# TiloccaS/DASemanticSegmentationAML

Measured on NVIDIA B200. Metric: da_train_step_img_per_s, higher is better.
Workload: dtype bf16

## Files before the change

dasemanticsegmentationaml_b200/csrc/igemm.cu:

```cuda
#include <stdlib.h>
#include <string.h>
#include <mutex>

#include "igemm.cuh"
#include "ptx.cuh"
#include "status.h"
#include "b200seg.h"

namespace b200 {

constexpr int kThreads = 192;
constexpr int kMaxStages = 8;

struct PipeBarriers {
  uint64_t full[kMaxStages];
  uint64_t empty[kMaxStages];
  uint64_t accum;
  uint32_t tmem_base;
};

__device__ __forceinline__ float apply_act(float v, int act, float slope) {
  if (act == 1) return fmaxf(v, 0.f);
  if (act == 2) return fmaf(slope, fminf(v, 0.f), fmaxf(v, 0.f));
  return v;
}

__device__ __forceinline__ void store16(const ConvParams& p, size_t off, const float (&v)[16]) {
  if (p.out_f32) {
    float* o = reinterpret_cast<float*>(p.out) + off;
    if (p.wide) {
#pragma unroll
      for (int h = 0; h < 2; ++h) {
        uint32_t r[8];
#pragma unroll
        for (int j = 0; j < 8; ++j) r[j] = __float_as_uint(v[8 * h + j]);
        st_global_v8(o + 8 * h, r);
      }
    } else {
#pragma unroll
      for (int j = 0; j < 4; ++j)
        reinterpret_cast<float4*>(o)[j] = make_float4(v[4 * j], v[4 * j + 1], v[4 * j + 2], v[4 * j + 3]);
    }
  } else {
    __nv_bfloat16* o = reinterpret_cast<__nv_bfloat16*>(p.out) + off;
// ... 777 lines not shown
    if (mark) dbg_mark(p, 8 + 4 * lt + 2);
    const int h = tc.h0 + rank * p.th + hl, w = tc.w0 + wl;
    const PairClass kc = cls[z];
    const bool valid = (h < kc.Ho) && (w < kc.Wo);
    const bool all_valid = __all_sync(0xffffffffu, valid);
    const size_t pix =
        ((size_t)tc.n_img * p.Hout + (size_t)(h * p.os + kc.oa)) * p.Wout + (w * p.os + kc.ob);
    const size_t obase = pix * p.out_ld + p.out_coff + tc.n0;
    StoreCoord sc;
    sc.map = tma_out ? &om.m[z] : nullptr;
    sc.w = tc.w0 + ws;
    sc.h = tc.h0 + rank * p.th + hs;
    sc.n = tc.n_img;
#ifdef B200_EPI_PREFETCH
    uint32_t r[32], rn[32];
    tmem_ld32(acc + c0, r);
#else
    uint32_t r[32];
#endif
#pragma unroll 1
    for (int b = 0; b < nb; ++b) {
      const int c = c0 + cstep * b;
#ifndef B200_EPI_PREFETCH
      tmem_ld32(acc + c, r);
#endif
      tmem_ld_wait32(r);
      if (b + 1 < nb) {
#ifdef B200_EPI_PREFETCH
        tmem_ld32(acc + c + cstep, rn);
#endif
      } else {
        tc_fence_before();
        __syncwarp();
        if (lane == 0) mbar_arrive_leader(smem_u32(&bars.tempty[buf]));
        if (mark) dbg_mark(p, 8 + 4 * lt + 3);
      }
      if (b == 0 && mark && lt == 1) dbg_mark(p, 4);
      uint64_t bs = 0ull, bq = 0ull;
      sc.c = tc.n0 + c;
      epilogue_batch32<F32, STATS>(p, r, valid, all_valid, obase + c, pix, tc.n0 + c, ns, tb, sc, bs, bq, lane);
      if (STATS) {
#pragma unroll
        for (int k = 0; k < 4; ++k) {
          a_sum[k] = f32x2_add(a_sum[k], b == k ? bs : 0ull);
          a_sq[k] = f32x2_add(a_sq[k], b == k ? bq : 0ull);
        }
      }
      if (b == 0 && mark && lt == 1) dbg_mark(p, 5);
#ifdef B200_EPI_PREFETCH
      if (b + 1 < nb) {
#pragma unroll
        for (int j = 0; j < 32; ++j) r[j] = rn[j];
      }
#endif
    }
    if (mark && lt == 1) dbg_mark(p, 6);
  }
  if (STATS && cur_n0 >= 0) {
    fold_stats();
    asm volatile("bar.sync 1, 256;" ::: "memory");
    flush_add_v4(p.stats + cur_n0, s_stats[0], p.BN, t, 256);
    if (!p.stats_sum_only) flush_add_v4(p.stats + p.stats_ld + cur_n0, s_stats[1], p.BN, t, 256);
  }
  if (tma_out && lane == 0) bulk_wait_read_all();
}

__global__ void __cluster_dims__(2, 1, 1) __launch_bounds__(kPairThreads, 1)
conv_igemm_pair_kernel(const __grid_constant__ CUtensorMap tmA, const __grid_constant__ CUtensorMap tmB,
                       const __grid_constant__ OutMaps om, const __grid_constant__ ConvParams p, int m_total,
                       int n_tiles, int n_slabs) {
  extern __shared__ uint8_t smem_raw[];
  __shared__ PairBarriers bars;
  __shared__ float s_stats[2][256];
  __shared__ __align__(1024) float s_tr[8][kTrWords];
  __shared__ uint32_t s_tapA[kMaxClasses][kMaxTaps + 1], s_tapB[kMaxClasses][kMaxTaps + 1], s_tapK[kMaxClasses][kMaxTaps + 1];
  __shared__ PairClass s_cls[kMaxClasses];
  __shared__ int s_pl[4][2];
  __shared__ int s_tapD[kMaxClasses][kMaxTaps][2];

  const int warp = threadIdx.x >> 5;
  const int lane = threadIdx.x & 31;
  const int rank = (int)cluster_ctarank();
  const bool leader = rank == 0;
  const int pair = blockIdx.x >> 1, n_pairs = gridDim.x >> 1;
  if (threadIdx.x == 0 && blockIdx.x == 0) dbg_mark(p, 0);
  const uint32_t smem_base = (smem_u32(smem_raw) + 1023u) & ~1023u;
  const uint32_t a_bytes = 128u * p.KC * 2u;
  const uint32_t b_half = (uint32_t)(p.BN / 2) * p.KC * 2u;
  const uint32_t stage_bytes = (uint32_t)p.kg * (a_bytes + b_half);
  const uint32_t plane_tx = (uint32_t)p.box_h * p.box_w * p.KC * 2u;
  const uint32_t plane_bytes = (plane_tx + 1023u) & ~1023u;
  const uint32_t halo_bytes = (uint32_t)p.np * plane_bytes;
  const uint32_t bslot_bytes = (uint32_t)p.tb * b_half;
  const uint32_t bring_base = smem_base + (uint32_t)p.stages * halo_bytes;
  const int cin_blocks = p.cin_pad / p.KC;
  const int my_n = pair % n_tiles;
  const int m_slots = n_pairs / n_tiles, m_slot = pair / n_tiles;
// ... 297 lines not shown
            } else {
#pragma unroll
              for (int k = 0; k < 2; ++k) {
                umma_f16_pair(acc, ((uint64_t)d_hi << 32) | (a_lo + 2u * k), ((uint64_t)d_hi << 32) | (b_lo + 2u * k), idesc, accum);
                accum = 1u;
              }
            }
            a_lo += a_bytes >> 4;
            b_lo += b_half >> 4;
          }
          umma_commit_pair(empty0 + 8u * s, 3);
          if (++s == p.stages) {
            s = 0;
            ph ^= 1u;
          }
          ready = mbar_try_wait(full0 + 8u * s, ph);
        }
        umma_commit_pair(smem_u32(&bars.tfull[buf]), 3);
        if (dbg_on && lt < kDbgTiles) dbg_mark(p, 8 + 4 * lt + 1);
      }
      }
    }
  } else {
    float* tb = &s_tr[warp - 2][0];
    if (p.out_f32) {
      if (p.stats != nullptr) pair_epilogue<true, true>(p, om, s_cls, bars, s_stats, tb, tmem, rank, my_n, m_first, m_stop, warp, lane);
      else pair_epilogue<true, false>(p, om, s_cls, bars, s_stats, tb, tmem, rank, my_n, m_first, m_stop, warp, lane);
    } else {
      if (p.stats != nullptr) pair_epilogue<false, true>(p, om, s_cls, bars, s_stats, tb, tmem, rank, my_n, m_first, m_stop, warp, lane);
      else pair_epilogue<false, false>(p, om, s_cls, bars, s_stats, tb, tmem, rank, my_n, m_first, m_stop, warp, lane);
    }
  }

  tc_fence_before();
  __syncthreads();
  cluster_sync_all();
  if (warp == 1) {
    tc_fence_after();
    tmem_dealloc_pair(tmem, tmem_cols);
  }
  if (threadIdx.x == 0 && blockIdx.x == 0) dbg_mark(p, 3);
}

__global__ void __launch_bounds__(kThreads, 1)
wgrad_igemm_kernel(const __grid_constant__ CUtensorMap tmDZ, const __grid_constant__ CUtensorMap tmX,
                   const __grid_constant__ WgradParams p) {
  extern __shared__ uint8_t smem_raw[];
  __shared__ PipeBarriers bars;

  const int warp = threadIdx.x >> 5;
  const int lane = threadIdx.x & 31;

  int y = blockIdx.y;
  const int ci_t = y % p.ci_tiles;
  y /= p.ci_tiles;
  const int co_t = y % p.co_tiles;
  const int tap = y / p.co_tiles;
  const int co0 = co_t * 128, ci0 = ci_t * p.BNW;

  const int tiles_per_img = p.tiles_h * p.tiles_w;
  const int total_tiles = tiles_per_img * p.n_img;
  const int per_split = (total_tiles + p.splits - 1) / p.splits;
  const int tile_begin = blockIdx.x * per_split;
  const int tile_end = min(total_tiles, tile_begin + per_split);
  const int nk = tile_end - tile_begin;
  if (nk <= 0) return;
// ... 607 lines not shown
  const size_t total = (size_t)rows_pad * RS * inner_pad;
  int blocks = (int)((total + 255) / 256);
  if (blocks > 148 * 8) blocks = 148 * 8;
  if (blocks < 1) blocks = 1;
  pack_filter_kernel<<<blocks, 256, 0, stream>>>(w, static_cast<__nv_bfloat16*>(out_bf16), Cout, Cin,
                                                 RS, rows_pad, inner_pad, transpose);
  return check_launch("pack_filter");
}

int b200_pack_filters_batched(const int64_t* table_dev, int n_filters, cudaStream_t stream) {
  if (n_filters <= 0) return B200_OK;
  pack_filters_batched_kernel<<<dim3(148, n_filters), 256, 0, stream>>>(
      reinterpret_cast<const long long*>(table_dev));
  return check_launch("pack_filters_batched");
}

static int g_debug_knob = 0;
int b200_debug_knob(int knob) {
  g_debug_knob = knob;
  return B200_OK;
}
static long long* g_debug_timeline = nullptr;
int b200_debug_timeline(int64_t* buf) {
  g_debug_timeline = reinterpret_cast<long long*>(buf);
  return B200_OK;
}

int b200_wgrad_unscratch_pairview(const float* scratch, float* dw, int Cout, int Cin, cudaStream_t stream) {
  if (Cin > 32 || Cout < 1) return set_error(B200_EINVAL, "wgrad_unscratch_pairview: needs Cin <= 32");
  wgrad_unscratch_pairview_kernel<<<(Cout * Cin * 16 + 255) / 256, 256, 0, stream>>>(scratch, dw, Cout, Cin);
  return check_launch("wgrad_unscratch_pairview");
}

int b200_conv_igemm(const void* in, int in_ld, int in_coff, int in_C, int N, int Hin, int Win,
                    const void* filt, int filt_rows, int cin_pad, int n_slabs,
                    void* out, int out_ld, int out_coff, int Hout, int Wout, int out_f32,
                    int n_classes, const int* class_Ho, const int* class_Wo, const int* class_oa,
                    const int* class_ob, const int* class_ntaps, const int* taps, int taps_stride,
                    int in_stride, int out_stride, const float* bias, int act, float slope,
                    float* stats, int stats_ld, const void* mask, int mask_ld, float mask_slope,
                    int stats_sum_only, int tune, cudaStream_t stream) {
  int pair_mode = (tune >> 22) & 1;
  int auto_taps = 0;
  for (int z = 0; z < n_classes && z < kMaxClasses; ++z) auto_taps = class_ntaps[z] > auto_taps ? class_ntaps[z] : auto_taps;
  const bool thin_auto = tune == 0 && cin_pad == 32 && auto_taps >= 9;
  if (tune == 0 && filt_rows % 32 == 0 && !thin_auto) pair_mode = 1;
  const int bn_override = tune & 0xFFF, mt_override = pair_mode ? 2 : (tune >> 12) & 0xF, st_override = (tune >> 16) & 0xF;
  if (n_classes < 1 || n_classes > kMaxClasses) return set_error(B200_EINVAL, "conv_igemm: bad class count %d", n_classes);
  if (cin_pad % 32) return set_error(B200_EINVAL, "conv_igemm: cin_pad %d not a multiple of 32", cin_pad);
  if (in_ld % 8 || in_coff % 8 || out_ld % 8 || out_coff % 8)
    return set_error(B200_EINVAL, "conv_igemm: channel strides/offsets must be multiples of 8");
  if (filt_rows % 16) return set_error(B200_EINVAL, "conv_igemm: filter rows %d not a multiple of 16", filt_rows);
  if (mask != nullptr && (mask_ld % 8 || (reinterpret_cast<uintptr_t>(mask) & 15)))
    return set_error(B200_EINVAL, "conv_igemm: the mask view must be 16-byte aligned with a pixel stride that is a multiple of 8");
  if (stats != nullptr && ((reinterpret_cast<uintptr_t>(stats) & 15) || stats_ld % 4))
    return set_error(B200_EINVAL, "conv_igemm: the statistics buffer must be 16-byte aligned with a row length that is a multiple of 4");
  if (bias != nullptr && (reinterpret_cast<uintptr_t>(bias) & 15))
    return set_error(B200_EINVAL, "conv_igemm: the bias vector must be 16-byte aligned");
  int rc = ensure_smem_optin();
  if (rc) return rc;

  ConvParams p;
  memset(&p, 0, sizeof(p));
  p.KC = (cin_pad % 64 == 0) ? 64 : 32;
  int max_wo = 0;
  for (int z = 0; z < n_classes; ++z) max_wo = class_Wo[z] > max_wo ? class_Wo[z] : max_wo;
  pick_patch(max_wo, &p.th, &p.tw, 128);
  int halo_mode = (tune >> 23) & 1;
  bool halo_ok = pair_mode && (in_stride == 1 || in_stride == 2);
  int min_taps = kMaxTaps;
  if (halo_ok) {
    const int s = in_stride;
    int cl_min[4], n_cl = 0;
    if (s == 1) {
// ... 222 lines not shown
        fits = sa * halo_slot + bring <= dyn;
      } else {
        if (st_override < 2 && 3 * halo_slot + 2 * tb * b_half > dyn) sa = 2;
        while (tb > 1 && sa * halo_slot + 2 * tb * b_half > dyn) tb = fix_tb(tb - 1);
        fits = sa * halo_slot + 2 * tb * b_half <= dyn;
        if (fits) {
          sb = (int)((dyn - sa * halo_slot) / (tb * b_half));
          if (sb > kMaxStages) sb = kMaxStages;
          bring = (size_t)sb * tb * b_half;
        }
      }
      if (sa > kMaxStages) sa = kMaxStages;
      if (!fits) {
        if ((tune >> 23) & 1) return set_error(B200_EINVAL, "conv_igemm: halo rings do not fit shared memory at BN = %d", p.BN);
        p.halo = 0;
      } else {
        p.tb = tb;
        p.sb = sb;
        p.stages = sa;
        p.kg = 1;
        rc = make_act_map(&tmA, in, in_coff, in_C, in_ld, N, Hin, Win, p.KC, p.box_w, p.box_h, in_stride, p.KC * 2);
        if (rc) return rc;
        rc = make_filter_map(&tmB, filt, filt_rows, n_slabs * cin_pad, p.KC, p.BN / 2, p.KC * 2);
        if (rc) return rc;
        int m_total = 0;
        for (int z = 0; z < n_classes; ++z) m_total += p.tiles_h[z] * p.tiles_w[z] * N;
        const int n_tiles = filt_rows / p.BN;
        const int total_tiles = m_total * n_tiles;
        const size_t psmem = sa * halo_slot + bring + 1024;
        int pairs = max_active_pairs(psmem);
        if (pairs > total_tiles) pairs = total_tiles;
        pairs = (pairs / n_tiles) * n_tiles;
        if (pairs < n_tiles) pairs = n_tiles;
        conv_igemm_pair_kernel<<<2 * pairs, kPairThreads, psmem, stream>>>(tmA, tmB, om, p, m_total, n_tiles, n_slabs);
        return check_launch("conv_igemm(pair, halo)");
      }
    }
    auto kg_divides = [&](int k) {
      for (int z = 0; z < n_classes; ++z)
        if ((class_ntaps[z] * cin_blocks) % k) return false;
      return true;
    };
    while (kg > 1 && (!kg_divides(kg) || 3 * kg * (128 * p.KC * 2 + (p.BN / 2) * p.KC * 2) > kPairDyn)) --kg;
    p.kg = kg;
    const int pstage = kg * (128 * p.KC * 2 + (p.BN / 2) * p.KC * 2);
    int st = st_override >= 2 ? st_override : kPairDyn / pstage;
    if (st > kMaxStages) st = kMaxStages;
    while (st > 2 && st * pstage > kPairDyn) --st;
    if (st < 2 || st * pstage > kPairDyn) return set_error(B200_EINVAL, "conv_igemm: pair tile does not fit shared memory");
    p.stages = st;
    rc = make_act_map(&tmA, in, in_coff, in_C, in_ld, N, Hin, Win, p.KC, p.tw, p.th, in_stride, p.KC * 2);
    if (rc) return rc;
    rc = make_filter_map(&tmB, filt, filt_rows, n_slabs * cin_pad, p.KC, p.BN / 2, p.KC * 2);
    if (rc) return rc;
    int m_total = 0;
    for (int z = 0; z < n_classes; ++z) m_total += p.tiles_h[z] * p.tiles_w[z] * N;
    const int n_tiles = filt_rows / p.BN;
    const int total_tiles = m_total * n_tiles;
    const size_t psmem = (size_t)p.stages * pstage + 1024;
    int pairs = max_active_pairs(psmem);
    if (pairs > total_tiles) pairs = total_tiles;
    pairs = (pairs / n_tiles) * n_tiles;
    if (pairs < n_tiles) pairs = n_tiles;
    conv_igemm_pair_kernel<<<2 * pairs, kPairThreads, psmem, stream>>>(tmA, tmB, om, p, m_total, n_tiles, n_slabs);
    return check_launch("conv_igemm(pair)");
  }
  rc = make_act_map(&tmA, in, in_coff, in_C, in_ld, N, Hin, Win, p.KC, p.tw, p.th * p.mt, in_stride, p.KC * 2);
  if (rc) return rc;
  rc = make_filter_map(&tmB, filt, filt_rows, n_slabs * cin_pad, p.KC, p.BN, p.KC * 2);
  if (rc) return rc;

  size_t smem = (size_t)p.stages * stage_bytes + 1024;
  const int persist = (tune >> 20) & 1;
  int b_res = (tune >> 21) & 1;
  const size_t bres_bytes = (size_t)n_slabs * cin_pad * p.BN * 2;
  if (b_res && (!persist || bres_bytes > 128 * 1024)) b_res = 0;
  if (b_res) {
    const int a_stage = p.mt * 128 * p.KC * 2;
    while (p.stages > 2 && bres_bytes + (size_t)p.stages * a_stage > 208 * 1024) --p.stages;
    if (bres_bytes + (size_t)p.stages * a_stage > 208 * 1024) b_res = 0;
    else smem = bres_bytes + (size_t)p.stages * a_stage + 1024;
  }
  if (persist && 2 * p.mt * p.BN <= 512) {
    int m_total = 0;
    for (int z = 0; z < n_classes; ++z) m_total += p.tiles_h[z] * p.tiles_w[z] * N;
    const int total_tiles = m_total * (filt_rows / p.BN);
    int per_sm = (int)((227 * 1024 - 4096) / (smem + 9 * 1024));
    const int tmem_need = 2 * p.mt * p.BN <= 32 ? 32 : (2 * p.mt * p.BN <= 64 ? 64 : (2 * p.mt * p.BN <= 128 ? 128 : (2 * p.mt * p.BN <= 256 ? 256 : 512)));
    if (per_sm > 512 / tmem_need) per_sm = 512 / tmem_need;
    if (per_sm > 4) per_sm = 4;
    if (per_sm < 1) per_sm = 1;
    int grid_p = 148 * per_sm;
    if (grid_p > total_tiles) grid_p = total_tiles;
    const int n_tiles = filt_rows / p.BN;
    grid_p = (grid_p / n_tiles) * n_tiles;
    if (grid_p < n_tiles) grid_p = n_tiles;
    conv_igemm_persistent_kernel<<<grid_p, kThreads, smem, stream>>>(tmA, tmB, p, m_total, n_tiles, b_res, n_slabs);
    return check_launch("conv_igemm(persistent)");
  }
  dim3 grid(max_tiles, filt_rows / p.BN, n_classes);
  conv_igemm_kernel<<<grid, kThreads, smem, stream>>>(tmA, tmB, p);
  return check_launch("conv_igemm");
}

int b200_conv_wgrad(const void* dz, int dz_ld, int dz_coff, int Cout, int N, int Ho, int Wo,
                    const void* x, int x_ld, int x_coff, int Cin, int Hin, int Win,
                    int n_taps, const int* taps , int RS,
                    int in_stride, float* dw, float* scratch, int ci_pad, int tune, cudaStream_t stream) {
  const int bnw_override = tune & 0xFFF, st_override = (tune >> 12) & 0xF;
  const int sp_override = (tune >> 16) & 0xFFF, kp_override = (tune >> 28) & 0x3;
  if (n_taps < 1 || n_taps > kMaxTaps) return set_error(B200_EINVAL, "conv_wgrad: bad tap count");
  if (dz_ld % 8 || dz_coff % 8 || x_ld % 8 || x_coff % 8)
    return set_error(B200_EINVAL, "conv_wgrad: channel strides/offsets must be multiples of 8");
  int rc = ensure_smem_optin();
  if (rc) return rc;
  WgradParams p;
  memset(&p, 0, sizeof(p));
  if (scratch != nullptr && (ci_pad % 16 || ci_pad < Cin || (reinterpret_cast<uintptr_t>(scratch) & 15)))
    return set_error(B200_EINVAL, "conv_wgrad: scratch needs 16-byte alignment and ci_pad = round_up(Cin, 16)");
  if (scratch != nullptr && Cin <= 32)
    return set_error(B200_EINVAL, "conv_wgrad: the tap-major scratch is for Cin > 32 (thin layers use the all-taps kernel)");
  if (Cin <= 32 && n_taps * 32 <= 512 && n_taps >= 16 && kp_override != 3 && (int64_t)N * Ho * Wo >= 262144) {
    TapPlanes tpl;
    const bool planes = kp_override == 1 && plan_planes(taps, n_taps, in_stride, &tpl);
    if (planes) {
      p.th = 8;
      p.tw = 8;
      p.np = tpl.np;
      p.box_h = p.th + tpl.eh;
      p.box_w = p.tw + tpl.ew;
      for (int q = 0; q < 4; ++q) {
        p.pl_dh[q] = tpl.pl_dh[q];
        p.pl_dw[q] = tpl.pl_dw[q];
      }
      for (int t = 0; t < n_taps; ++t) {
// ... 123 lines not shown
```

dasemanticsegmentationaml_b200/csrc/igemm.cuh:

```cuda
#pragma once
#include <stdint.h>

namespace b200 {

constexpr int kMaxTaps = 16;
constexpr int kMaxClasses = 4;

struct ConvParams {
  int Ho[kMaxClasses], Wo[kMaxClasses];
  int tiles_h[kMaxClasses], tiles_w[kMaxClasses];
  int n_taps[kMaxClasses];
  int8_t tap_dh[kMaxClasses][kMaxTaps];
  int16_t tap_dw[kMaxClasses][kMaxTaps];
  int8_t tap_k[kMaxClasses][kMaxTaps];
  int oa[kMaxClasses], ob[kMaxClasses];
  int n_img;
  int th, tw;
  int mt;
  int in_stride;
  int cin_pad;
  int KC;
  int BN;
  int stages;
  void* out;
  int out_ld;
  int out_coff;
  int Hout, Wout;
  int os;
  const float* bias;
  int act;
  float slope;
  int out_f32;
  float* stats;
  int stats_ld;
  const void* mask;
  int mask_ld;
  float mask_slope;
  int stats_sum_only;
  int wide;
  int kg;
  int halo;
  int np;
  int box_h, box_w;
  int pl_dh[4], pl_dw[4];
  int8_t tap_pl[kMaxClasses][kMaxTaps];
  int8_t tap_off[kMaxClasses][kMaxTaps];
  int tb, sb;
  int bres;
  int tma_out;
  long long* dbg;
  int dbg_knob;
};

struct WgradParams {
  int Ho, Wo, tiles_h, tiles_w, n_img;
  int th, tw;
  int in_stride;
  int n_taps;
  int8_t tap_dh[kMaxTaps];
  int16_t tap_dw[kMaxTaps];
  int RS;
  int8_t tap_rs[kMaxTaps];
  int Cout, Cin;
  int co_tiles, ci_tiles;
  int BNW;
  int stages;
  int splits;
  float* dw;
  float* scratch;
  int ci_pad;
  int np, box_h, box_w;
  int pl_dh[4], pl_dw[4];
  int8_t tap_pl[kMaxTaps];
  int8_t tap_off[kMaxTaps];
};

struct TapPlanes {
  int np, eh, ew;
  int pl_dh[4], pl_dw[4];
  int8_t tap_pl[kMaxTaps];
  int8_t tap_qh[kMaxTaps], tap_qw[kMaxTaps];
};
// ... 3 lines not shown
```

dasemanticsegmentationaml_b200/kernels.py:

```python
import ctypes

import torch

from . import _lib
from ._lib import c_float, c_int, c_int64, call, check, int_array, lib, ptr, stream


def round_up(v, m):
    return (v + m - 1) // m * m


def _nhwc_meta(t):
    assert t.dim() == 4 and t.stride(3) == 1, "expected an NHWC tensor with unit channel stride"
    n, h, w, c = t.shape
    ld = t.stride(2)
    assert t.stride(1) == w * ld and t.stride(0) == h * w * ld, "NHWC view must be pixel-dense"
    return n, h, w, c, ld


def pack_filter(weight, transpose=False, rows_pad=None):
    cout, cin, r, s = weight.shape
    rows, inner = (cin, cout) if transpose else (cout, cin)
    rows_pad = round_up(rows, 16) if rows_pad is None else rows_pad
    assert rows_pad >= rows and rows_pad % 16 == 0
# ... 91 lines not shown
        half = (w + 2) // 2
        classes = [dict(Ho=(h + 2) // 2, Wo=half, oa=0, ob=r * half,
                        taps=[(-a, -b, (2 * a + r) * 2 + b) for a in range(2) for b in range(2)]) for r in range(2)]
        g = _geom_cache[key] = Geometry(classes, 1, 1, (h + 2) // 2, w + 2, "pvd4x4s2p1")
    return g


TUNED = {}
RECORD = None


def load_tuned(path=None):
    import json
    import os
    path = path or os.path.join(os.path.dirname(os.path.abspath(__file__)), "tuned_tiles.json")
    if os.path.exists(path):
        with open(path) as f:
            TUNED.update({k: int(v) for k, v in json.load(f).items()})


load_tuned()


def conv_key(n, hin, win, cin_pad, rows_pad, geom, f32, stats, mask=False):
    return "conv %d %d %d c%d r%d %s%s%s%s" % (n, hin, win, cin_pad, rows_pad, geom.key, " f32" if f32 else "",
                                                " st" if stats else "", " mk" if mask else "")


def wgrad_key(n, ho, wo, cout, cin, r, s, stride):
    return "wgrad %d %d %d co%d ci%d %dx%ds%d" % (n, ho, wo, cout, cin, r, s, stride)


def conv_igemm(x, filt, out, geom, bias=None, act=0, slope=0.0, stats=None, bn_tile=None, k_real=None, n_real=None,
               mask=None, mask_slope=0.0, stats_sum_only=False):
    n, hin, win, cin, in_ld = _nhwc_meta(x)
    n2, hout, wout, cout_view, out_ld = _nhwc_meta(out)
    rows_pad, n_slabs, cin_pad = filt.shape
    assert n2 == n and hout == geom.Hout and wout == geom.Wout, "output shape mismatch"
    assert cout_view == rows_pad, "output view must expose exactly the packed filter's rows"
    assert x.dtype == torch.bfloat16 and filt.dtype == torch.bfloat16
    out_f32 = 1 if out.dtype == torch.float32 else 0
    if not out_f32:
        assert out.dtype == torch.bfloat16
    if stats is not None:
        assert stats.dtype == torch.float32 and stats.dim() == 2 and stats.shape[0] == 2
    if mask is not None:
        assert mask.dtype == torch.bfloat16 and tuple(mask.shape[:3]) == (n, hout, wout) and mask.shape[3] >= rows_pad
    flops = 2.0 * geom.px_taps * n * (k_real or min(cin, cin_pad)) * (n_real or rows_pad)
    if bn_tile is None:
        key = conv_key(n, hin, win, cin_pad, rows_pad, geom, out_f32, stats is not None and not stats_sum_only, mask is not None)
        bn_tile = TUNED.get(key, 0)
        if RECORD is not None:
            RECORD.append(("conv", key, dict(n=n, hin=hin, win=win, cin=cin, in_ld=in_ld, rows=rows_pad, cin_pad=cin_pad,
                                              n_slabs=n_slabs, geom=geom, f32=out_f32, stats=stats is not None,
                                              bias=bias is not None, out_ld=out_ld, flops=flops, mask=mask is not None,
                                              sum_only=bool(stats_sum_only))))
    call("b200_conv_igemm",
         ptr(x), c_int(in_ld), c_int(0), c_int(cin), c_int(n), c_int(hin), c_int(win),
         ptr(filt), c_int(rows_pad), c_int(cin_pad), c_int(n_slabs),
         ptr(out), c_int(out_ld), c_int(0), c_int(hout), c_int(wout), c_int(out_f32),
         geom.c_n, geom.c_ho, geom.c_wo, geom.c_oa, geom.c_ob, geom.c_nt, geom.c_taps, c_int(geom.tmax),
         c_int(geom.in_stride), c_int(geom.out_stride), ptr(bias), c_int(act), c_float(slope),
         ptr(stats), c_int(0 if stats is None else stats.shape[1]),
         ptr(mask), c_int(0 if mask is None else mask.stride(2)), c_float(mask_slope), c_int(1 if stats_sum_only else 0),
         c_int(bn_tile), stream(), flops=flops,
         tag="M%d N%d K%dx%d s%d/%d%s" % (n * geom.classes[0]["Ho"] * geom.classes[0]["Wo"] * len(geom.classes), rows_pad, cin_pad,
                                            len(geom.classes[0]["taps"]), geom.in_stride, geom.out_stride, " stats" if stats is not None else ""))
    return out


_wgrad_taps = {}


def conv_wgrad(dz, x, dw, r, s, stride, pad, tune=None, scratch=None, taps=None, flops=None, tune_cout=None):
    n, ho, wo, _, dz_ld = _nhwc_meta(dz)
    n2, hin, win, _, x_ld = _nhwc_meta(x)
    cout, cin = dw.shape[0], dw.shape[1]
    assert n2 == n and dw.dtype == torch.float32 and dw.is_contiguous()
    tkey = (r, s, pad) if taps is None else tuple(taps)
    taps_c = _wgrad_taps.get(tkey)
    if taps_c is None:
        flat = []
        if taps is None:
            for i in range(r):
                for j in range(s):
                    flat += [i - pad, j - pad, i * s + j]
        else:
            assert len(taps) == r * s
            for t in taps:
                flat += list(t)
        taps_c = _wgrad_taps[tkey] = int_array(flat)
    tap_list, taps = taps, taps_c
    if tune is None:
        key = wgrad_key(n, ho, wo, cout if tune_cout is None else tune_cout, cin, r, s, stride) + ("" if tap_list is None else " v%d" % max(t[1] for t in tap_list))
        tune = TUNED.get(key, 0)
        if RECORD is not None:
            RECORD.append(("wgrad", key, dict(n=n, ho=ho, wo=wo, cout=cout, cin=cin, r=r, s=s, stride=stride, pad=pad,
# ... 319 lines not shown
```

dasemanticsegmentationaml_b200/ops.py:

```python
import torch

from . import kernels as K

BF16 = torch.bfloat16
F32 = torch.float32

FORCE_REPACK = False


def packed_filter(weight, transpose, shape=None, rows_pad=None):
    cache = getattr(weight, "_b200_pack", None)
    if cache is None:
        cache = {}
        try:
            weight._b200_pack = cache
        except AttributeError:
            pass
    shape = tuple(shape) if shape is not None else tuple(weight.shape)
    key = (int(transpose), shape)
    ver, ptr_now = weight._version, weight.data_ptr()
    hit = cache.get(key)
    if hit is not None and hit[0] == ver and hit[1] == ptr_now and not FORCE_REPACK:
        return hit[2]
    w = weight.detach().view(shape)
# ... 169 lines not shown
        for key, comm in self.streams.items():
            torch.cuda.current_stream(torch.device("cuda", key)).wait_stream(comm)
        left = []
        for g in grads:
            ptr = g.data_ptr()
            if not (g.dtype == F32 and any(lo <= ptr and ptr + 4 * g.numel() <= hi for lo, hi, _ in self.spans)):
                left.append(g)
        self.spans = []
        return left


REDUCER = _GradReducer()


def zeros_f32(shape, device):
    return ARENA.zeros(tuple(shape) if not isinstance(shape, int) else (shape,), device)


def empty_act(n, h, w, c, device):
    return torch.empty((n, h, w, c), dtype=BF16, device=device)


class BNCtx:
    __slots__ = ("z", "scale", "shift", "mean", "rstd", "act", "slope", "training")


def bn_act_fwd(z, stats, bn, training, act, slope=0.0, out=None):
    n, h, w, c = z.shape
    gamma, beta, rm, rv = bn
    buf = torch.empty((4, c), dtype=F32, device=z.device)
    a = out if out is not None else torch.empty_like(z)
    K.bn_norm_act(z, a, stats, float(n * h * w), gamma, beta, rm, rv, training, act, slope,
                  buf[0], buf[1], buf[2], buf[3])
    ctx = BNCtx()
    ctx.z, ctx.scale, ctx.shift, ctx.mean, ctx.rstd = z, buf[0], buf[1], buf[2], buf[3]
    ctx.act, ctx.slope, ctx.training = act, slope, training
    return a, ctx


def bn_act_bwd(ctx, dy1, dy2=None):
    if not ctx.training:
        raise NotImplementedError("backward through eval-mode BatchNorm is not part of the reference's training path")
    c = ctx.z.shape[3]
    red = zeros_f32((1 + K.BN_RED_REPLICAS, 2, c), ctx.z.device)
    dz = torch.empty(ctx.z.shape, dtype=BF16, device=ctx.z.device)
    K.bn_act_bwd_fused(dy1, dy2, ctx.z, dz, ctx.scale, ctx.shift, ctx.mean, ctx.rstd, red, ctx.act, ctx.slope)
    return dz, red[0, 1], red[0, 0]


class ConvCtx:
    __slots__ = ("x", "weight", "stride", "pad", "bn", "a", "act", "slope", "stem_col")


def conv_raw_fwd(x, weight, stride, pad, stats=None, bias=None, act=K.ACT_NONE, slope=0.0, out=None,
                 out_dtype=BF16, rows_pad=None):
    n, h, w, _ = x.shape
    _, _, r, s = weight.shape
    geom = K.fwd_geometry(h, w, r, s, stride, pad)
    filt = packed_filter(weight, False, rows_pad=rows_pad)
    if out is None:
        out = torch.empty((n, geom.Hout, geom.Wout, filt.shape[0]), dtype=out_dtype, device=x.device)
    K.conv_igemm(x, filt, out, geom, bias=bias, act=act, slope=slope, stats=stats,
                 k_real=weight.shape[1], n_real=weight.shape[0])
    return out


def conv_dgrad(dz, weight, stride, pad, hin, win, mask=None, mask_slope=0.0, dbias=None):
    _, _, r, s = weight.shape
    geom = K.dgrad_geometry(hin, win, r, s, stride, pad)
    filt_t = packed_filter(weight, True)
# ... 96 lines not shown
            self.keep = []


SIDE = _SideStream()
WGRAD_SIDE_MAX_PIXELS = 65536


def conv_wgrad(dz, x, weight, stride, pad, tune_cout=None):
    cout, cin, r, s = weight.shape
    dw = zeros_f32((cout, cin, r, s), dz.device)
    scratch = WSCRATCH.request(dw, cout, cin, r * s)
    if WSCRATCH.depth > 0 and dz.shape[0] * dz.shape[1] * dz.shape[2] <= WGRAD_SIDE_MAX_PIXELS:
        SIDE.run(dz.device, (dz, x, dw, scratch),
                 lambda: K.conv_wgrad(dz, x, dw, r, s, stride, pad, scratch=scratch, tune_cout=tune_cout))
    else:
        K.conv_wgrad(dz, x, dw, r, s, stride, pad, scratch=scratch, tune_cout=tune_cout)
    return dw


def conv_bn_act_fwd(x, weight, bn, stride, pad, training, act=K.ACT_RELU, slope=0.0, out=None):
    cout = weight.shape[0]
    stats = zeros_f32((2, cout), weight.device) if training else None
    ctx = ConvCtx()
    ctx.stem_col = None
    if x.dim() == 4 and x.dtype == F32 and x.shape[1] == 3 and weight.shape[1] == 3:
        assert weight.shape[2] == 3 and stride == 2 and pad == 1 and cout == 32
        n, _, h, w = x.shape
        ho, wo = (h - 1) // 2 + 1, (w - 1) // 2 + 1
        col = K.stem_im2col(x, empty_act(n, ho, wo, 32, x.device))
        z = empty_act(n, ho, wo, cout, x.device)
        K.conv_igemm(col, packed_filter(weight, False, (cout, 27, 1, 1)), z, K.fwd_geometry(ho, wo, 1, 1, 1, 0),
                     stats=stats, k_real=27, n_real=cout)
        ctx.stem_col = col
    else:
        assert cout % 16 == 0, "BatchNorm'd convs have a multiple of 16 output channels"
        z = conv_raw_fwd(x, weight, stride, pad, stats=stats)
    a, bnctx = bn_act_fwd(z, stats, bn, training, act, slope, out)
    ctx.x, ctx.weight, ctx.stride, ctx.pad, ctx.bn, ctx.a = x, weight, stride, pad, bnctx, a
    ctx.act, ctx.slope = act, slope
    return a, ctx


def conv_bn_act_bwd(ctx, dy1, dy2=None, need_dx=True):
    dz, dgamma, dbeta = bn_act_bwd(ctx.bn, dy1, dy2)
    if ctx.stem_col is not None:
        dw = zeros_f32(ctx.weight.shape, dz.device)
        K.conv_wgrad(dz, ctx.stem_col[..., :27], dw.view(dw.shape[0], 27, 1, 1), 1, 1, 1, 0)
        return None, dw, dgamma, dbeta
    dw = conv_wgrad(dz, ctx.x, ctx.weight, ctx.stride, ctx.pad)
    dx = None
    if need_dx:
        dx = conv_dgrad(dz, ctx.weight, ctx.stride, ctx.pad, ctx.x.shape[1], ctx.x.shape[2])
    return dx, dw, dgamma, dbeta


class ConvBiasCtx:
    __slots__ = ("x", "weight", "stride", "pad", "a", "act", "slope", "has_bias", "pairview")


def conv_pairview_fwd(xpad, weight, bias_padded, act, slope):
    n, hp, wp, c = xpad.shape
    assert c == 32 and xpad.is_contiguous() and hp % 2 == 0 and wp % 2 == 0
    h, w = hp - 2, wp - 2
    cout, cin = weight.shape[0], weight.shape[1]
    xv = xpad.view(n, hp // 2, wp, 64)
    a = torch.empty((n, h // 2, w // 2, cout), dtype=BF16, device=xpad.device)
    K.conv_igemm(xv, packed_filter_pairview(weight, False), a, K.pairview_fwd_geometry(h, w), bias=bias_padded, act=act,
                 slope=slope, k_real=2 * cin, n_real=cout)
    ctx = ConvBiasCtx()
    ctx.x, ctx.weight, ctx.stride, ctx.pad, ctx.a, ctx.act, ctx.slope = xv, weight, 2, 1, a, act, slope
# ... 163 lines not shown
```

include/b200seg.h:

```cpp
#ifndef B200SEG_H_
#define B200SEG_H_

#include <stddef.h>
#include <stdint.h>

#ifndef __DRIVER_TYPES_H__
typedef struct CUstream_st* cudaStream_t;
#endif

#define B200_OK 0
#define B200_EINVAL (-1)
#define B200_ECUDA (-2)
#define B200_EDRIVER (-3)
#define B200_EARCH (-4)

#ifdef __cplusplus
extern "C" {
#endif

const char* b200_last_error(void);
int b200_version(void);
int b200_check_device(void);

int b200_pack_filter(const float* w, void* out_bf16, int Cout, int Cin, int RS, int rows_pad,
                     int inner_pad, int transpose, cudaStream_t stream);

int b200_pack_filters_batched(const int64_t* table_dev, int n_filters, cudaStream_t stream);

int b200_conv_igemm(const void* in, int in_ld, int in_coff, int in_C, int N, int Hin, int Win,
                    const void* filt, int filt_rows, int cin_pad, int n_slabs, void* out, int out_ld,
                    int out_coff, int Hout, int Wout, int out_f32, int n_classes, const int* class_Ho,
                    const int* class_Wo, const int* class_oa, const int* class_ob,
                    const int* class_ntaps, const int* taps, int taps_stride, int in_stride,
                    int out_stride, const float* bias, int act, float slope, float* stats,
                    int stats_ld, const void* mask, int mask_ld, float mask_slope, int stats_sum_only,
                    int tune, cudaStream_t stream);

int b200_debug_timeline(int64_t* buf);
int b200_debug_knob(int knob);

int b200_conv_wgrad(const void* dz, int dz_ld, int dz_coff, int Cout, int N, int Ho, int Wo,
                    const void* x, int x_ld, int x_coff, int Cin, int Hin, int Win, int n_taps,
                    const int* taps, int RS, int in_stride, float* dw, float* scratch, int ci_pad, int tune,
                    cudaStream_t stream);
int b200_wgrad_unscratch(const float* scratch_base, float* dw_base, const int64_t* table_dev, int n_layers,
                         cudaStream_t stream);
int b200_wgrad_unscratch_pairview(const float* scratch, float* dw, int Cout, int Cin, cudaStream_t stream);

int b200_stem_im2col(const float* img, int N, int H, int W, void* col, int col_ld, cudaStream_t stream);

int b200_channel_stats(const void* x, int ld, int C, int64_t npix, float* stats, cudaStream_t stream);
int b200_bn_finalize(const float* stats, int C, float count, const float* gamma, const float* beta,
                     float* running_mean, float* running_var, float momentum, float eps,
                     int training, float* scale, float* shift, float* mean_out, float* rstd_out,
                     cudaStream_t stream);
int b200_bn_act_apply(const void* x, int x_ld, void* y, int y_ld, int C, int64_t npix,
                      const float* scale, const float* shift, int act, float slope,
                      cudaStream_t stream);
int b200_bn_norm_act(const void* x, int x_ld, void* y, int y_ld, int C, int64_t npix,
                     const float* stats, float count, const float* gamma, const float* beta,
                     float* running_mean, float* running_var, float momentum, float eps,
                     int training, int act, float slope, float* scale, float* shift,
                     float* mean_out, float* rstd_out, cudaStream_t stream);
int b200_bn_act_bwd_reduce(const void* dy1, int dy1_ld, const void* dy2, int dy2_ld, const void* z,
                           int z_ld, int C, int64_t npix, const float* scale, const float* shift,
                           const float* mean, const float* rstd, int act, float slope, float* red,
                           cudaStream_t stream);
int b200_bn_act_bwd_apply(const void* dy1, int dy1_ld, const void* dy2, int dy2_ld, const void* z,
                          int z_ld, void* dz, int dz_ld, int C, int64_t npix, const float* scale,
// ... 98 lines not shown
```

Baseline: 715.1.

## Fuse training BatchNorm+activation into conv kernel via cooperative grid sync

When the whole conv fits in one wave, the pair conv kernel is launched cooperatively. It keeps accumulators resident in tensor memory, grid-syncs after the per-channel statistics are reduced, then computes BN coefficients and running stats and writes the normalized, activated bf16 output straight from TMEM. This removes the separate bn_norm_act pass that re-reads z from global memory. In exchange it adds a grid-wide barrier and tries several tile candidates, falling back to the unfused path when no one-wave plan exists. Holding TMEM buffers for the whole kernel may also limit overlap.

Result: no change. 720.3 (median of 6 runs) (+0.7%).

```diff
diff --git a/dasemanticsegmentationaml_b200/csrc/igemm.cu b/dasemanticsegmentationaml_b200/csrc/igemm.cu
--- a/dasemanticsegmentationaml_b200/csrc/igemm.cu
+++ b/dasemanticsegmentationaml_b200/csrc/igemm.cu
@@ -1,6 +1,8 @@
 #include <stdlib.h>
 #include <string.h>
 #include <mutex>
+
+#include <cooperative_groups.h>
 
 #include "igemm.cuh"
 #include "ptx.cuh"
@@ -10,6 +12,9 @@
 namespace b200 {
 
 constexpr int kThreads = 192;
+constexpr int kNotOneWave = 1;
+constexpr int kKnobNoBnFold = 1 << 6;
+constexpr int kKnobBnFoldOnly = 1 << 7;
 constexpr int kMaxStages = 8;
 
 struct PipeBarriers {
@@ -853,7 +858,7 @@
       } else {
         tc_fence_before();
         __syncwarp();
-        if (lane == 0) mbar_arrive_leader(smem_u32(&bars.tempty[buf]));
+        if (lane == 0 && !p.bn_fold) mbar_arrive_leader(smem_u32(&bars.tempty[buf]));
         if (mark) dbg_mark(p, 8 + 4 * lt + 3);
       }
       if (b == 0 && mark && lt == 1) dbg_mark(p, 4);
@@ -884,6 +889,72 @@
     if (!p.stats_sum_only) flush_add_v4(p.stats + p.stats_ld + cur_n0, s_stats[1], p.BN, t, 256);
   }
   if (tma_out && lane == 0) bulk_wait_read_all();
+}
+
+__device__ __forceinline__ void pair_bn_apply(const ConvParams& p, const PairClass* cls, const float (*s_coef)[256],
+                                              uint32_t tmem, int rank, int my_n, int m_first, int m_stop, int warp,
+                                              int lane) {
+  const int q = warp & 3;
+  const int half = (warp - 2) >> 2;
+  const bool alt = p.BN <= kPairAltBN;
+  const int row = q * 32 + lane;
+  const int hl = row / p.tw, wl = row - hl * p.tw;
+  const float ns = p.bn_act == 0 ? 1.f : (p.bn_act == 1 ? 0.f : p.bn_slope);
+  const int c0 = alt ? 0 : 32 * half;
+  const int cstep = alt ? 32 : 64;
+  const int nb = alt ? (p.BN >> 5) : (p.BN >> 6);
+  int lt = 0;
+  for (TileIter it(p, my_n, m_first, m_stop); it.valid(); it.next(p), ++lt) {
+    if (alt && (lt & 1) != half) continue;
+    const TileCoord tc = it.coord(p);
+    const uint32_t acc = tmem + (uint32_t)(lt * p.BN) + ((uint32_t)(q * 32) << 16);
+    const int h = tc.h0 + rank * p.th + hl, w = tc.w0 + wl;
+    const PairClass kc = cls[tc.z];
+    const bool valid = (h < kc.Ho) && (w < kc.Wo);
+    const size_t pix = ((size_t)tc.n_img * p.Hout + (size_t)(h * p.os + kc.oa)) * p.Wout + (w * p.os + kc.ob);
+    __nv_bfloat16* o = reinterpret_cast<__nv_bfloat16*>(p.bn_out) + pix * p.bn_out_ld + tc.n0;
+#pragma unroll 1
+    for (int b = 0; b < nb; ++b) {
+      const int c = c0 + cstep * b;
+      uint32_t r[32];
+      tmem_ld32(acc + c, r);
+      tmem_ld_wait32(r);
+      if (!valid) continue;
+      uint32_t pk[16];
+#pragma unroll
+      for (int j = 0; j < 16; ++j) {
+        const float2 z = unpack_bf16(pack_bf16(__uint_as_float(r[2 * j]), __uint_as_float(r[2 * j + 1])));
+        const float v0 = fmaf(z.x, s_coef[0][c + 2 * j], s_coef[1][c + 2 * j]);
+        const float v1 = fmaf(z.y, s_coef[0][c + 2 * j + 1], s_coef[1][c + 2 * j + 1]);
+        pk[j] = pack_bf16(fmaf(ns, fminf(v0, 0.f), fmaxf(v0, 0.f)), fmaf(ns, fminf(v1, 0.f), fmaxf(v1, 0.f)));
+      }
+      if (p.bn_wide) {
+        uint32_t q8[8];
+#pragma unroll
+        for (int hv = 0; hv < 2; ++hv) {
+#pragma unroll
+          for (int j = 0; j < 8; ++j) q8[j] = pk[8 * hv + j];
+          st_global_v8(o + c + 16 * hv, q8);
+        }
+      } else {
+#pragma unroll
+        for (int j = 0; j < 4; ++j)
+          reinterpret_cast<uint4*>(o + c)[j] = make_uint4(pk[4 * j], pk[4 * j + 1], pk[4 * j + 2], pk[4 * j + 3]);
+      }
+    }
+  }
+}
+
+__device__ __forceinline__ void bn_fold_coeffs(const ConvParams& p, int c, float* mean, float* var, float* rstd,
+                                               float* sc, float* sh) {
+  const float s1 = __ldcg(p.stats + c), s2 = __ldcg(p.stats + p.stats_ld + c);
+  const float g = p.bn_gamma != nullptr ? p.bn_gamma[c] : 1.f;
+  const float be = p.bn_beta != nullptr ? p.bn_beta[c] : 0.f;
+  *mean = __fdiv_rn(s1, p.bn_count);
+  *var = fmaxf(__fdiv_rn(s2, p.bn_count) - *mean * *mean, 0.f);
+  *rstd = rsqrtf(*var + p.bn_eps);
+  *sc = g * *rstd;
+  *sh = be - *mean * g * *rstd;
 }
 
 __global__ void __cluster_dims__(2, 1, 1) __launch_bounds__(kPairThreads, 1)
@@ -1247,6 +1318,39 @@
     }
   }
 
+  if (p.bn_fold) {
+    cooperative_groups::this_grid().sync();
+    if (warp >= 2) {
+      const int t = threadIdx.x - 64;
+      const int n0 = my_n * p.BN;
+      for (int col = t; col < p.BN; col += 256) {
+        float mean, var, rstd, sc, sh;
+        bn_fold_coeffs(p, n0 + col, &mean, &var, &rstd, &sc, &sh);
+        s_stats[0][col] = sc;
+        s_stats[1][col] = sh;
+      }
+      if (blockIdx.x == 0) {
+        const int C = p.stats_ld;
+        for (int c = t; c < C; c += 256) {
+          float mean, var, rstd, sc, sh;
+          bn_fold_coeffs(p, c, &mean, &var, &rstd, &sc, &sh);
+          p.bn_coef[c] = sc;
+          p.bn_coef[C + c] = sh;
+          p.bn_coef[2 * C + c] = mean;
+          p.bn_coef[3 * C + c] = rstd;
+          if (p.bn_rmean != nullptr) {
+            const float unbiased = p.bn_count > 1.f ? __fdiv_rn(var * p.bn_count, p.bn_count - 1.f) : var;
+            p.bn_rmean[c] = (1.f - p.bn_momentum) * p.bn_rmean[c] + p.bn_momentum * mean;
+            p.bn_rvar[c] = (1.f - p.bn_momentum) * p.bn_rvar[c] + p.bn_momentum * unbiased;
+          }
+        }
+      }
+      asm volatile("bar.sync 1, 256;" ::: "memory");
+      tc_fence_after();
+      pair_bn_apply(p, s_cls, s_stats, tmem, rank, my_n, m_first, m_stop, warp, lane);
+    }
+  }
+
   tc_fence_before();
   __syncthreads();
   cluster_sync_all();
@@ -1920,14 +2024,66 @@
   return check_launch("wgrad_unscratch_pairview");
 }
 
-int b200_conv_igemm(const void* in, int in_ld, int in_coff, int in_C, int N, int Hin, int Win,
-                    const void* filt, int filt_rows, int cin_pad, int n_slabs,
-                    void* out, int out_ld, int out_coff, int Hout, int Wout, int out_f32,
-                    int n_classes, const int* class_Ho, const int* class_Wo, const int* class_oa,
-                    const int* class_ob, const int* class_ntaps, const int* taps, int taps_stride,
-                    int in_stride, int out_stride, const float* bias, int act, float slope,
-                    float* stats, int stats_ld, const void* mask, int mask_ld, float mask_slope,
-                    int stats_sum_only, int tune, cudaStream_t stream) {
+}
+
+namespace b200 {
+
+static int launch_bn_fold(const CUtensorMap& tmA, const CUtensorMap& tmB, const OutMaps& om, ConvParams p,
+                          const ConvParams& bf, int m_total, int n_tiles, int n_slabs, int pairs, size_t psmem,
+                          cudaStream_t stream) {
+  const int m_slots = pairs / n_tiles;
+  const int per_pair = (m_total + m_slots - 1) / m_slots;
+  if (per_pair > (p.BN <= 128 ? 4 : 2) || (p.dbg_knob & kKnobNoBnFold)) return kNotOneWave;
+  p.bn_fold = 1;
+  p.bn_out = bf.bn_out;
+  p.bn_out_ld = bf.bn_out_ld;
+  p.bn_wide = bf.bn_wide;
+  p.bn_gamma = bf.bn_gamma;
+  p.bn_beta = bf.bn_beta;
+  p.bn_rmean = bf.bn_rmean;
+  p.bn_rvar = bf.bn_rvar;
+  p.bn_count = bf.bn_count;
+  p.bn_momentum = bf.bn_momentum;
+  p.bn_eps = bf.bn_eps;
+  p.bn_act = bf.bn_act;
+  p.bn_slope = bf.bn_slope;
+  p.bn_coef = bf.bn_coef;
+  cudaLaunchConfig_t cfg;
+  memset(&cfg, 0, sizeof(cfg));
+  cfg.gridDim = dim3(2 * pairs, 1, 1);
+  cfg.blockDim = dim3(kPairThreads, 1, 1);
+  cfg.dynamicSmemBytes = psmem;
+  cfg.stream = stream;
+  cudaLaunchAttribute attr[2];
+  attr[0].id = cudaLaunchAttributeCooperative;
+  attr[0].val.cooperative = 1;
+  attr[1].id = cudaLaunchAttributeClusterDimension;
+  attr[1].val.clusterDim.x = 2;
+  attr[1].val.clusterDim.y = 1;
+  attr[1].val.clusterDim.z = 1;
+  cfg.attrs = attr;
+  cfg.numAttrs = 2;
+  cudaError_t e = cudaLaunchKernelEx(&cfg, conv_igemm_pair_kernel, tmA, tmB, om, p, m_total, n_tiles, n_slabs);
+  if (e != cudaSuccess) {
+    (void)cudaGetLastError();
+    cfg.numAttrs = 1;
+    e = cudaLaunchKernelEx(&cfg, conv_igemm_pair_kernel, tmA, tmB, om, p, m_total, n_tiles, n_slabs);
+  }
+  if (e != cudaSuccess) {
+    (void)cudaGetLastError();
+    return kNotOneWave;
+  }
+  return check_launch("conv_igemm(pair, one-wave BatchNorm)");
+}
+
+static int conv_igemm_impl(const void* in, int in_ld, int in_coff, int in_C, int N, int Hin, int Win,
+                           const void* filt, int filt_rows, int cin_pad, int n_slabs,
+                           void* out, int out_ld, int out_coff, int Hout, int Wout, int out_f32,
+                           int n_classes, const int* class_Ho, const int* class_Wo, const int* class_oa,
+                           const int* class_ob, const int* class_ntaps, const int* taps, int taps_stride,
+                           int in_stride, int out_stride, const float* bias, int act, float slope,
+                           float* stats, int stats_ld, const void* mask, int mask_ld, float mask_slope,
+                           int stats_sum_only, int tune, const ConvParams* bf, cudaStream_t stream) {
   int pair_mode = (tune >> 22) & 1;
   int auto_taps = 0;
   for (int z = 0; z < n_classes && z < kMaxClasses; ++z) auto_taps = class_ntaps[z] > auto_taps ? class_ntaps[z] : auto_taps;
@@ -2216,6 +2372,7 @@
         if (pairs > total_tiles) pairs = total_tiles;
         pairs = (pairs / n_tiles) * n_tiles;
         if (pairs < n_tiles) pairs = n_tiles;
+        if (bf != nullptr) return launch_bn_fold(tmA, tmB, om, p, *bf, m_total, n_tiles, n_slabs, pairs, psmem, stream);
         conv_igemm_pair_kernel<<<2 * pairs, kPairThreads, psmem, stream>>>(tmA, tmB, om, p, m_total, n_tiles, n_slabs);
         return check_launch("conv_igemm(pair, halo)");
       }
@@ -2246,9 +2403,11 @@
     if (pairs > total_tiles) pairs = total_tiles;
     pairs = (pairs / n_tiles) * n_tiles;
     if (pairs < n_tiles) pairs = n_tiles;
+    if (bf != nullptr) return launch_bn_fold(tmA, tmB, om, p, *bf, m_total, n_tiles, n_slabs, pairs, psmem, stream);
     conv_igemm_pair_kernel<<<2 * pairs, kPairThreads, psmem, stream>>>(tmA, tmB, om, p, m_total, n_tiles, n_slabs);
     return check_launch("conv_igemm(pair)");
   }
+  if (bf != nullptr) return kNotOneWave;
   rc = make_act_map(&tmA, in, in_coff, in_C, in_ld, N, Hin, Win, p.KC, p.tw, p.th * p.mt, in_stride, p.KC * 2);
   if (rc) return rc;
   rc = make_filter_map(&tmB, filt, filt_rows, n_slabs * cin_pad, p.KC, p.BN, p.KC * 2);
@@ -2285,6 +2444,72 @@
   dim3 grid(max_tiles, filt_rows / p.BN, n_classes);
   conv_igemm_kernel<<<grid, kThreads, smem, stream>>>(tmA, tmB, p);
   return check_launch("conv_igemm");
+}
+
+}
+
+extern "C" {
+
+int b200_conv_igemm(const void* in, int in_ld, int in_coff, int in_C, int N, int Hin, int Win,
+                    const void* filt, int filt_rows, int cin_pad, int n_slabs,
+                    void* out, int out_ld, int out_coff, int Hout, int Wout, int out_f32,
+                    int n_classes, const int* class_Ho, const int* class_Wo, const int* class_oa,
+                    const int* class_ob, const int* class_ntaps, const int* taps, int taps_stride,
+                    int in_stride, int out_stride, const float* bias, int act, float slope,
+                    float* stats, int stats_ld, const void* mask, int mask_ld, float mask_slope,
+                    int stats_sum_only, void* bn_out, int bn_out_ld, const float* bn_gamma, const float* bn_beta,
+                    float* bn_running_mean, float* bn_running_var, float bn_momentum, float bn_eps, int bn_act,
+                    float bn_slope, float* bn_coef, int tune, cudaStream_t stream) {
+  if (bn_out == nullptr)
+    return conv_igemm_impl(in, in_ld, in_coff, in_C, N, Hin, Win, filt, filt_rows, cin_pad, n_slabs, out, out_ld, out_coff,
+                           Hout, Wout, out_f32, n_classes, class_Ho, class_Wo, class_oa, class_ob, class_ntaps, taps,
+                           taps_stride, in_stride, out_stride, bias, act, slope, stats, stats_ld, mask, mask_ld, mask_slope,
+                           stats_sum_only, tune, nullptr, stream);
+  if (stats == nullptr || stats_sum_only || out_f32 || bias != nullptr || act != 0 || mask != nullptr || n_classes != 1 ||
+      out_stride != 1 || stats_ld != filt_rows || bn_coef == nullptr)
+    return set_error(B200_EINVAL, "conv_igemm: BatchNorm needs one class of plain bf16 outputs with statistics and coefficients");
+  if (bn_out_ld % 8 || (reinterpret_cast<uintptr_t>(bn_out) & 15))
+    return set_error(B200_EINVAL, "conv_igemm: the BatchNorm output view must be 16-byte aligned with a pixel stride that is a multiple of 8");
+  const int64_t npix = (int64_t)N * Hout * Wout;
+  ConvParams bf;
+  memset(&bf, 0, sizeof(bf));
+  bf.bn_out = bn_out;
+  bf.bn_out_ld = bn_out_ld;
+  bf.bn_wide = (reinterpret_cast<uintptr_t>(bn_out) & 31) == 0 && bn_out_ld % 16 == 0;
+  bf.bn_gamma = bn_gamma;
+  bf.bn_beta = bn_beta;
+  bf.bn_rmean = bn_running_mean;
+  bf.bn_rvar = bn_running_var;
+  bf.bn_count = (float)npix;
+  bf.bn_momentum = bn_momentum;
+  bf.bn_eps = bn_eps;
+  bf.bn_act = bn_act;
+  bf.bn_slope = bn_slope;
+  bf.bn_coef = bn_coef;
+  int cands[9], nc = 0;
+  cands[nc++] = tune;
+  for (int bn = 32; bn <= 256; bn <<= 1)
+    if (filt_rows % bn == 0 && bn >= (tune & 0xFFF)) {
+      if ((tune >> 23) & 1) cands[nc++] = (1 << 23) | (1 << 22) | bn;
+      cands[nc++] = (1 << 22) | bn;
+    }
+  for (int i = 0; i < nc; ++i) {
+    const int rc = conv_igemm_impl(in, in_ld, in_coff, in_C, N, Hin, Win, filt, filt_rows, cin_pad, n_slabs, out, out_ld,
+                                   out_coff, Hout, Wout, 0, 1, class_Ho, class_Wo, class_oa, class_ob, class_ntaps, taps,
+                                   taps_stride, in_stride, 1, nullptr, 0, 0.f, stats, stats_ld, nullptr, 0, 0.f, 0, cands[i],
+                                   &bf, stream);
+    if (rc == B200_OK) return rc;
+    if (rc != kNotOneWave && i == 0) return rc;
+  }
+  if (g_debug_knob & kKnobBnFoldOnly) return set_error(B200_EINVAL, "conv_igemm: no one-wave BatchNorm plan");
+  int rc = conv_igemm_impl(in, in_ld, in_coff, in_C, N, Hin, Win, filt, filt_rows, cin_pad, n_slabs, out, out_ld, out_coff,
+                           Hout, Wout, 0, 1, class_Ho, class_Wo, class_oa, class_ob, class_ntaps, taps, taps_stride,
+                           in_stride, 1, nullptr, 0, 0.f, stats, stats_ld, nullptr, 0, 0.f, 0, tune, nullptr, stream);
+  if (rc) return rc;
+  return b200_bn_norm_act(static_cast<const __nv_bfloat16*>(out) + out_coff, out_ld, bn_out, bn_out_ld, filt_rows, npix,
+                          stats, (float)npix, bn_gamma, bn_beta, bn_running_mean, bn_running_var, bn_momentum, bn_eps, 1,
+                          bn_act, bn_slope, bn_coef, bn_coef + filt_rows, bn_coef + 2 * filt_rows, bn_coef + 3 * filt_rows,
+                          stream);
 }
 
 int b200_conv_wgrad(const void* dz, int dz_ld, int dz_coff, int Cout, int N, int Ho, int Wo,
diff --git a/dasemanticsegmentationaml_b200/csrc/igemm.cuh b/dasemanticsegmentationaml_b200/csrc/igemm.cuh
--- a/dasemanticsegmentationaml_b200/csrc/igemm.cuh
+++ b/dasemanticsegmentationaml_b200/csrc/igemm.cuh
@@ -48,6 +48,17 @@
   int tb, sb;
   int bres;
   int tma_out;
+  int bn_fold;
+  void* bn_out;
+  int bn_out_ld, bn_wide;
+  const float* bn_gamma;
+  const float* bn_beta;
+  float* bn_rmean;
+  float* bn_rvar;
+  float bn_count, bn_momentum, bn_eps;
+  int bn_act;
+  float bn_slope;
+  float* bn_coef;
   long long* dbg;
   int dbg_knob;
 };
diff --git a/dasemanticsegmentationaml_b200/kernels.py b/dasemanticsegmentationaml_b200/kernels.py
--- a/dasemanticsegmentationaml_b200/kernels.py
+++ b/dasemanticsegmentationaml_b200/kernels.py
@@ -147,7 +147,7 @@
 
 
 def conv_igemm(x, filt, out, geom, bias=None, act=0, slope=0.0, stats=None, bn_tile=None, k_real=None, n_real=None,
-               mask=None, mask_slope=0.0, stats_sum_only=False):
+               mask=None, mask_slope=0.0, stats_sum_only=False, bn=None):
     n, hin, win, cin, in_ld = _nhwc_meta(x)
     n2, hout, wout, cout_view, out_ld = _nhwc_meta(out)
     rows_pad, n_slabs, cin_pad = filt.shape
@@ -162,6 +162,10 @@
     if mask is not None:
         assert mask.dtype == torch.bfloat16 and tuple(mask.shape[:3]) == (n, hout, wout) and mask.shape[3] >= rows_pad
     flops = 2.0 * geom.px_taps * n * (k_real or min(cin, cin_pad)) * (n_real or rows_pad)
+    bn_y, bn_g, bn_b, bn_rm, bn_rv, bn_act, bn_slope, bn_coef = bn if bn is not None else (None,) * 5 + (0, 0.0, None)
+    if bn is not None:
+        assert stats is not None and bn_y.dtype == torch.bfloat16 and tuple(bn_y.shape) == tuple(out.shape)
+        assert bn_coef.dtype == torch.float32 and bn_coef.is_contiguous() and tuple(bn_coef.shape) == (4, rows_pad)
     if bn_tile is None:
         key = conv_key(n, hin, win, cin_pad, rows_pad, geom, out_f32, stats is not None and not stats_sum_only, mask is not None)
         bn_tile = TUNED.get(key, 0)
@@ -178,6 +182,8 @@
          c_int(geom.in_stride), c_int(geom.out_stride), ptr(bias), c_int(act), c_float(slope),
          ptr(stats), c_int(0 if stats is None else stats.shape[1]),
          ptr(mask), c_int(0 if mask is None else mask.stride(2)), c_float(mask_slope), c_int(1 if stats_sum_only else 0),
+         ptr(bn_y), c_int(0 if bn_y is None else bn_y.stride(2)), ptr(bn_g), ptr(bn_b), ptr(bn_rm), ptr(bn_rv),
+         c_float(0.1), c_float(1e-5), c_int(bn_act), c_float(bn_slope), ptr(bn_coef),
          c_int(bn_tile), stream(), flops=flops,
          tag="M%d N%d K%dx%d s%d/%d%s" % (n * geom.classes[0]["Ho"] * geom.classes[0]["Wo"] * len(geom.classes), rows_pad, cin_pad,
                                             len(geom.classes[0]["taps"]), geom.in_stride, geom.out_stride, " stats" if stats is not None else ""))
diff --git a/dasemanticsegmentationaml_b200/ops.py b/dasemanticsegmentationaml_b200/ops.py
--- a/dasemanticsegmentationaml_b200/ops.py
+++ b/dasemanticsegmentationaml_b200/ops.py
@@ -225,10 +225,14 @@
     a = out if out is not None else torch.empty_like(z)
     K.bn_norm_act(z, a, stats, float(n * h * w), gamma, beta, rm, rv, training, act, slope,
                   buf[0], buf[1], buf[2], buf[3])
+    return a, _bn_ctx(z, buf, act, slope, training)
+
+
+def _bn_ctx(z, coef, act, slope, training):
     ctx = BNCtx()
-    ctx.z, ctx.scale, ctx.shift, ctx.mean, ctx.rstd = z, buf[0], buf[1], buf[2], buf[3]
+    ctx.z, ctx.scale, ctx.shift, ctx.mean, ctx.rstd = z, coef[0], coef[1], coef[2], coef[3]
     ctx.act, ctx.slope, ctx.training = act, slope, training
-    return a, ctx
+    return ctx
 
 
 def bn_act_bwd(ctx, dy1, dy2=None):
@@ -391,10 +395,22 @@
         K.conv_igemm(col, packed_filter(weight, False, (cout, 27, 1, 1)), z, K.fwd_geometry(ho, wo, 1, 1, 1, 0),
                      stats=stats, k_real=27, n_real=cout)
         ctx.stem_col = col
+    elif training:
+        assert cout % 16 == 0, "BatchNorm'd convs have a multiple of 16 output channels"
+        n, h, w, _ = x.shape
+        geom = K.fwd_geometry(h, w, weight.shape[2], weight.shape[3], stride, pad)
+        filt = packed_filter(weight, False)
+        z = empty_act(n, geom.Hout, geom.Wout, filt.shape[0], x.device)
+        a = out if out is not None else torch.empty_like(z)
+        coef = torch.empty((4, cout), dtype=F32, device=x.device)
+        K.conv_igemm(x, filt, z, geom, stats=stats, k_real=weight.shape[1], n_real=cout,
+                     bn=(a, bn[0], bn[1], bn[2], bn[3], act, slope, coef))
+        bnctx = _bn_ctx(z, coef, act, slope, training)
     else:
         assert cout % 16 == 0, "BatchNorm'd convs have a multiple of 16 output channels"
         z = conv_raw_fwd(x, weight, stride, pad, stats=stats)
-    a, bnctx = bn_act_fwd(z, stats, bn, training, act, slope, out)
+    if ctx.stem_col is not None or not training:
+        a, bnctx = bn_act_fwd(z, stats, bn, training, act, slope, out)
     ctx.x, ctx.weight, ctx.stride, ctx.pad, ctx.bn, ctx.a = x, weight, stride, pad, bnctx, a
     ctx.act, ctx.slope = act, slope
     return a, ctx
diff --git a/include/b200seg.h b/include/b200seg.h
--- a/include/b200seg.h
+++ b/include/b200seg.h
@@ -34,7 +34,9 @@
                     const int* class_ntaps, const int* taps, int taps_stride, int in_stride,
                     int out_stride, const float* bias, int act, float slope, float* stats,
                     int stats_ld, const void* mask, int mask_ld, float mask_slope, int stats_sum_only,
-                    int tune, cudaStream_t stream);
+                    void* bn_out, int bn_out_ld, const float* bn_gamma, const float* bn_beta,
+                    float* bn_running_mean, float* bn_running_var, float bn_momentum, float bn_eps,
+                    int bn_act, float bn_slope, float* bn_coef, int tune, cudaStream_t stream);
 
 int b200_debug_timeline(int64_t* buf);
 int b200_debug_knob(int knob);
```
